# dropbox/divans

Measured on AMD Instinct MI355X. Metric: MB/s encode+decode per GPU, 64 KiB metablocks; bit-exact vs CPU, higher is better.
Workload: dtype u16/u64 integer

## Files before the change

divans_amd/csrc/capi.cpp:

```cpp
#include <hip/hip_runtime.h>

#include <algorithm>
#include <atomic>
#include <cstdio>
#include <cstdlib>
#include <cstring>
#include <mutex>
#include <string>
#include <vector>

#include "../../include/divans_gpu.h"
#include "lit_kernels.h"
#include "lit_device.h"

using namespace divans_hip;

static thread_local std::string g_last_error;
static int fail(int code, const std::string& msg) { g_last_error = msg; return code; }
#define HIP_TRY(expr)                                                                              \
    do {                                                                                           \
        hipError_t e_ = (expr);                                                                    \
        if (e_ != hipSuccess)                                                                      \
            return fail(DIVANS_GPU_EHIP, std::string(#expr) + ": " + hipGetErrorString(e_));       \
    } while (0)
// ... 916 lines not shown
            rc = after(s0, k.n_streams, view); if (rc) return rc;
        }
        return 0;
    }
    rc = ensure_sf(c, n_streams); if (rc) return rc;
    rc = ensure_tables(c); if (rc) return rc;
    LitBatch b;
    std::memset(&b, 0, sizeof(b));
    b.blob = c->d_blob; b.geom = c->geom; b.tables = c->d_tables;
    b.n_streams = n_streams; b.stream_len = stream_len; b.max_stream_len = c->max_stream_len;
    b.in = d_in; b.in_offsets = d_in_offsets; b.in_sizes = d_in_sizes;
    b.sf = c->d_sf; b.status = c->d_status;
    b.seg_begin = d_seg_begin; b.segs = (const LitSegment*)d_segs;
    set_cache_fields(c, b);
    if (d_segs && b.cache_mode != 2u && b.cache_mode != 0u) return fail(DIVANS_GPU_EINVAL, "segment lists need the default (high-nibble-row) cache or none");
    HIP_TRY(hipEventRecord(c->ev[0], c->stream));
    ++c->table_launch_seq;
    HIP_TRY(launch_model_encode(b, c->mix, c->blocks, c->stream));
    view.sf = c->d_sf; view.stride = 2u * c->max_stream_len;
    return after(0u, n_streams, view);
}

static int rans_event_pair(divans_gpu_codec* c, size_t i, hipEvent_t*& pair) {
    while (c->ev_rans.size() < 2u * (i + 1u)) {
        hipEvent_t e = nullptr;
        HIP_TRY(hipEventCreate(&e));
        c->ev_rans.push_back(e);
    }
    pair = &c->ev_rans[2u * i];
    return 0;
}

static int rans_pass(divans_gpu_codec* c, const SfView& v, uint32_t count, uint32_t stream_len, const uint32_t* d_in_sizes, uint8_t* out, uint64_t out_base,
                     uint64_t out_slot, uint64_t* d_out_offsets, uint32_t* d_out_sizes, uint32_t* d_chunk_bytes, uint32_t max_chunks, size_t& pairs) {
    const bool chunk_lanes = c->max_stream_len > 32768u && c->max_stream_len <= 65536u;
    RansBatch r;
    r.sf = v.sf; r.sf_stride = v.stride; r.n_streams = count; r.stream_len = stream_len; r.max_stream_len = c->max_stream_len;
    r.in_sizes = d_in_sizes;
    r.out = out; r.out_base = out_base; r.out_slot = out_slot;
    r.out_offsets = d_out_offsets; r.out_sizes = d_out_sizes;
    r.status = c->d_status; r.chunk_bytes = d_chunk_bytes; r.max_chunks = max_chunks;
    r.scratch = nullptr; r.scratch_stride = 0; r.chunk0_sizes = nullptr;
    if (chunk_lanes) { int rr = ensure_rans_scratch(c, count, v, r); if (rr) return rr; }
    r.split_states = (c->rans_split == 2u || (c->rans_split == 0u && (uint64_t)count * 4u <= (uint64_t)c->num_cus * 4u * 64u)) ? 1u : 0u;
    hipEvent_t* pair = nullptr;
    int rr = rans_event_pair(c, pairs, pair); if (rr) return rr;
    HIP_TRY(hipEventRecord(pair[0], c->stream));
    HIP_TRY(launch_rans_encode(r, c->stream));
    HIP_TRY(hipEventRecord(pair[1], c->stream));
    ++pairs;
    return 0;
}

static int encode_batch_impl(divans_gpu_codec* c, const uint8_t* d_in, const uint64_t* d_in_offsets,
                             const uint32_t* d_in_sizes, uint32_t stream_len, uint32_t n_streams,
                             uint8_t* d_out, uint64_t out_slot, uint64_t* d_out_offsets, uint32_t* d_out_sizes,
                             uint32_t* d_chunk_bytes, uint32_t max_chunks,
                             const uint32_t* d_seg_begin = nullptr, const divans_lit_segment* d_segs = nullptr);

extern "C" int divans_gpu_lit_encode_batch(divans_gpu_codec* c, const uint8_t* d_in, const uint64_t* d_in_offsets,
                                           const uint32_t* d_in_sizes, uint32_t stream_len, uint32_t n_streams,
                                           uint8_t* d_out, uint64_t out_slot, uint64_t* d_out_offsets, uint32_t* d_out_sizes) {
    return encode_batch_impl(c, d_in, d_in_offsets, d_in_sizes, stream_len, n_streams, d_out, out_slot, d_out_offsets,
                             d_out_sizes, nullptr, 0);
}

static int encode_batch_impl(divans_gpu_codec* c, const uint8_t* d_in, const uint64_t* d_in_offsets,
                             const uint32_t* d_in_sizes, uint32_t stream_len, uint32_t n_streams,
                             uint8_t* d_out, uint64_t out_slot, uint64_t* d_out_offsets, uint32_t* d_out_sizes,
                             uint32_t* d_chunk_bytes, uint32_t max_chunks,
                             const uint32_t* d_seg_begin, const divans_lit_segment* d_segs) {
    if (!c || !d_in || !d_out || !d_out_offsets || !d_out_sizes) return fail(DIVANS_GPU_EINVAL, "null argument");
    if ((d_seg_begin == nullptr) != (d_segs == nullptr)) return fail(DIVANS_GPU_EINVAL, "seg_begin and segs go together");
    if (n_streams == 0) return 0;
    if ((d_in_offsets == nullptr) != (d_in_sizes == nullptr)) return fail(DIVANS_GPU_EINVAL, "offsets and sizes go together");
    if (stream_len > c->max_stream_len) return fail(DIVANS_GPU_EINVAL, "stream_len exceeds the codec's max_stream_len");
// ... 11 lines not shown
    c->rans_pairs = pairs; c->enc_spans = 0;
    c->timing_pending_enc = true;
    return 0;
}

extern "C" int divans_gpu_lit_encode_packed(divans_gpu_codec* c, const uint8_t* d_in, const uint64_t* d_in_offsets, const uint32_t* d_in_sizes,
                                            uint32_t stream_len, uint32_t n_streams, uint8_t* d_packed, uint64_t packed_cap,
                                            uint64_t* d_packed_offsets, uint32_t* d_sizes, uint64_t* d_total, uint32_t sub_batch) {
    if (!c || !d_in || !d_packed || !d_packed_offsets || !d_sizes || !d_total) return fail(DIVANS_GPU_EINVAL, "null argument");
    if ((d_in_offsets == nullptr) != (d_in_sizes == nullptr)) return fail(DIVANS_GPU_EINVAL, "offsets and sizes go together");
    if (stream_len > c->max_stream_len) return fail(DIVANS_GPU_EINVAL, "stream_len exceeds the codec's max_stream_len");
    HIP_TRY(hipSetDevice(c->device));
    HIP_TRY(hipMemsetAsync(d_total, 0, sizeof(uint64_t), c->stream));
    if (n_streams == 0) return 0;
    const uint64_t slot = divans_gpu_lit_encode_bound(d_in_sizes ? c->max_stream_len : stream_len);
    uint32_t sub = std::min(n_streams, sub_batch ? sub_batch : c->bucket_mix_batch);
    while ((uint64_t)sub * slot > ((uint64_t)1 << 36) && sub > 1024u) sub = (sub + 1u) / 2u;
    if ((size_t)sub * slot > c->slots_bytes) {
        if (c->d_slots) { HIP_TRY(hipStreamSynchronize(c->stream)); HIP_TRY(hipFree(c->d_slots)); c->d_slots = nullptr; c->slots_bytes = 0; }
        if (device_alloc((void**)&c->d_slots, (size_t)sub * slot) != hipSuccess) return fail(DIVANS_GPU_ENOMEM, "hipMalloc(output slots of a sub-batch) failed");
        c->slots_bytes = (size_t)sub * slot;
    }
    if (sub > c->slot_off_cap) {
        if (c->d_slot_off) { HIP_TRY(hipStreamSynchronize(c->stream)); HIP_TRY(hipFree(c->d_slot_off)); c->d_slot_off = nullptr; c->slot_off_cap = 0; }
        if (hipMalloc(&c->d_slot_off, (size_t)sub * sizeof(uint64_t)) != hipSuccess) return fail(DIVANS_GPU_ENOMEM, "hipMalloc(slot offsets) failed");
        c->slot_off_cap = sub;
    }
    const size_t n_sub = (n_streams + sub - 1u) / sub;
    while (c->ev_span.size() < 3u * n_sub) { hipEvent_t e = nullptr; HIP_TRY(hipEventCreate(&e)); c->ev_span.push_back(e); }
    size_t pairs = 0, span = 0;
    for (uint32_t b0 = 0; b0 < n_streams; b0 += sub, ++span) {
        const uint32_t m = std::min(sub, n_streams - b0);
        HIP_TRY(hipEventRecord(c->ev_span[3u * span], c->stream));
        int rc = model_pass(c, d_in_offsets ? d_in : d_in + (size_t)b0 * stream_len, d_in_offsets ? d_in_offsets + b0 : nullptr, d_in_sizes ? d_in_sizes + b0 : nullptr,
                            stream_len, m, nullptr, nullptr, [&](uint32_t first, uint32_t count, const SfView& v) -> int {
            return rans_pass(c, v, count, stream_len, d_in_sizes ? d_in_sizes + b0 + first : nullptr, c->d_slots + (uint64_t)first * slot, (uint64_t)first * slot, slot,
                             c->d_slot_off + first, d_sizes + b0 + first, nullptr, 0, pairs);
        });
        if (rc) return rc;
        HIP_TRY(hipEventRecord(c->ev_span[3u * span + 1u], c->stream));
        HIP_TRY(launch_pack(c->d_slots, c->d_slot_off, d_sizes + b0, m, d_packed, d_packed_offsets + b0, d_total, c->stream, true, packed_cap, c->d_status));
        HIP_TRY(hipEventRecord(c->ev_span[3u * span + 2u], c->stream));
    }
    c->rans_pairs = pairs; c->enc_spans = span;
    c->timing_pending_enc = true;
    return 0;
}

extern "C" int divans_gpu_lit_encode_batch_chunks(divans_gpu_codec* c, const uint8_t* d_in, const uint64_t* d_in_offsets,
                                                  const uint32_t* d_in_sizes, uint32_t stream_len, uint32_t n_streams,
                                                  uint8_t* d_out, uint64_t out_slot, uint64_t* d_out_offsets, uint32_t* d_out_sizes,
                                                  uint32_t* d_chunk_bytes, uint32_t max_chunks) {
    if (!d_chunk_bytes || max_chunks < (2u * (uint64_t)stream_len + 65535u) / 65536u) return fail(DIVANS_GPU_EINVAL, "max_chunks too small");
    return encode_batch_impl(c, d_in, d_in_offsets, d_in_sizes, stream_len, n_streams, d_out, out_slot, d_out_offsets, d_out_sizes,
                             d_chunk_bytes, max_chunks);
}

extern "C" int divans_gpu_lit_encode_segments_batch(divans_gpu_codec* c, const uint8_t* d_in, const uint64_t* d_in_offsets,
                                                    const uint32_t* d_in_sizes, uint32_t stream_len, uint32_t n_streams,
                                                    const uint32_t* d_seg_begin, const divans_lit_segment* d_segs,
                                                    uint8_t* d_out, uint64_t out_slot, uint64_t* d_out_offsets, uint32_t* d_out_sizes) {
    if (!d_seg_begin || !d_segs) return fail(DIVANS_GPU_EINVAL, "null segment list");
    return encode_batch_impl(c, d_in, d_in_offsets, d_in_sizes, stream_len, n_streams, d_out, out_slot, d_out_offsets,
                             d_out_sizes, nullptr, 0, d_seg_begin, d_segs);
}

extern "C" int divans_gpu_lit_model_batch(divans_gpu_codec* c, const uint8_t* d_in, const uint64_t* d_in_offsets,
                                          const uint32_t* d_in_sizes, uint32_t stream_len, uint32_t n_streams, uint32_t* d_pairs) {
    if (!c || !d_in || !d_pairs) return fail(DIVANS_GPU_EINVAL, "null argument");
    if (n_streams == 0) return 0;
    if ((d_in_offsets == nullptr) != (d_in_sizes == nullptr)) return fail(DIVANS_GPU_EINVAL, "offsets and sizes go together");
    if (stream_len > c->max_stream_len) return fail(DIVANS_GPU_EINVAL, "stream_len exceeds the codec's max_stream_len");
    HIP_TRY(hipSetDevice(c->device));
    const size_t row = (size_t)2u * c->max_stream_len * sizeof(uint32_t);
// ... 782 lines not shown
```

divans_amd/csrc/lit_kernels.h:

```cpp
#ifndef DIVANS_LIT_KERNELS_H_
#define DIVANS_LIT_KERNELS_H_
#include <hip/hip_runtime.h>
#include <stdint.h>

namespace divans_hip {

constexpr int LIT_THREADS = 256;
constexpr int RANS_THREADS = 64;

constexpr uint32_t LIT_BLOB_LUT1CLASS = 0;
constexpr uint32_t LIT_BLOB_CTXF = 256;
constexpr uint32_t LIT_CTXF_BYTES = 2048;
constexpr uint32_t LIT_MAX_BTYPES = 8;
constexpr uint32_t LIT_BLOB_MAX_BYTES = 256 + LIT_CTXF_BYTES * LIT_MAX_BTYPES + 8192;

struct LitGeometry {
    uint32_t nctx;
    uint32_t low_width;
    uint32_t plane0, plane1, plane2;
    uint32_t low_base;
    uint32_t cm_base;
    uint32_t total_rows;
    int32_t mm_uniform;
    int32_t ctx_const;
// ... 10 lines not shown
struct LitBatch {
    const uint8_t* blob;
    LitGeometry geom;
    int16_t* tables;
    uint32_t n_streams, stream_len, max_stream_len;
    const uint8_t* in; const uint64_t* in_offsets; const uint32_t* in_sizes;
    uint8_t* out; const uint64_t* out_offsets; const uint32_t* out_sizes;
    uint32_t* sf;
    uint32_t cache_rows_high;
    uint32_t cache_rows_low;
    uint32_t cache_mode;
    uint32_t cache_bytes_per_wg;
    const uint32_t* seg_begin;
    const LitSegment* segs;
    uint32_t* status;
    uint32_t dm_log2, dm_shift;
    uint8_t* stream_bad;
    uint32_t resume; int32_t* wstate;
    uint32_t* consumed;
    const uint8_t* byte_rank;
};
constexpr uint32_t LIT_STATUS_BAD_MODEL = 1u;
constexpr uint32_t LIT_STATUS_BAD_SEGMENT = 4u;
constexpr uint32_t LIT_STATUS_OUTPUT_FULL = 8u;
constexpr uint32_t LIT_STATUS_BAD_STREAM = 2u;

struct RansBatch {
    const uint32_t* sf; uint32_t n_streams, stream_len, max_stream_len; const uint32_t* in_sizes;
    uint32_t sf_stride;
    uint64_t out_base;
    uint8_t* out; uint64_t out_slot; uint64_t* out_offsets; uint32_t* out_sizes; uint32_t* status;
    uint32_t* chunk_bytes; uint32_t max_chunks;
    uint8_t* scratch; uint64_t scratch_stride; uint32_t* chunk0_sizes;
    uint32_t split_states;
};

typedef unsigned int bk_u32x2 __attribute__((ext_vector_type(2)));
struct BucketBatch {
    const uint8_t* in; const uint64_t* in_offsets; const uint32_t* in_sizes;
    uint32_t n_streams, stream_len, max_stream_len;
    uint32_t pieces;
    uint32_t slot;
    uint32_t sf_stride;
    uint8_t* sorted;
    uint16_t* inv;
    uint32_t* desc;
    bk_u32x2* sfs;
    uint32_t* sf;
    uint32_t* tasks;
    uint32_t* counters;
    int32_t inc, lim;
};
hipError_t launch_bucket_model(const BucketBatch& b, uint32_t chain_blocks, hipStream_t st);
void launch_bucket_tasks(const BucketBatch& b, hipStream_t st);
void launch_bucket_unsort(const BucketBatch& b, hipStream_t st);
void launch_bucket_unsort32(const BucketBatch& b, hipStream_t st);

struct MixBucketBatch {
    const uint8_t* in; const uint64_t* in_offsets; const uint32_t* in_sizes;
    uint32_t n_streams, stream_len, max_stream_len;
    uint32_t pieces;
    uint32_t slot;
    uint32_t pos_stride;
    uint32_t sf_stride;
    const uint8_t* blob;
    uint16_t* sorted;
    uint16_t* inv;
    uint32_t* desc;
    uint32_t* tasks;
    uint32_t* counters;
    bk_u32x2* xs[2];
    uint32_t* maxes[2];
    uint32_t* sf;
    int32_t inc0, lim0, inc2, lim2, inc3, lim3;
};
hipError_t launch_bucket_mix_model(const MixBucketBatch& b, uint32_t num_cus, hipStream_t st);

uint32_t lit_lds_bytes(const LitBatch& b);
hipError_t launch_model_encode(const LitBatch& b, bool mix, uint32_t blocks, hipStream_t st);
hipError_t launch_rans_encode(const RansBatch& b, hipStream_t st);
hipError_t launch_decode(const LitBatch& b, bool mix, uint32_t blocks, hipStream_t st);
hipError_t launch_decode2(const LitBatch& b, bool mix, uint32_t blocks, hipStream_t st);
void lit_decode_kernel_name(const LitBatch& b, bool mix, char* buf, size_t cap);
void lit_decode2_kernel_name(const LitBatch& b, bool mix, char* buf, size_t cap);
uint32_t lit_decode2_effective_caches(uint32_t dm_log2, bool mix, bool seg);
uint32_t lit_decode2_stream_lds(uint32_t dm_log2);
#ifndef DIVANS_WITH_EXPERIMENTAL_DECODERS
#define DIVANS_WITH_EXPERIMENTAL_DECODERS 0
#endif
#if DIVANS_WITH_EXPERIMENTAL_DECODERS
hipError_t launch_decode_t(const LitBatch& b, bool mix, uint32_t blocks, hipStream_t st);
hipError_t launch_selftest_cdf_ops_t(const uint32_t* d_ops, uint32_t n, int32_t* d_out, hipStream_t st);
void lit_decode_t_kernel_name(const LitBatch& b, bool mix, char* buf, size_t cap);
uint32_t lit_decode_t_stream_lds(uint32_t dm_log2, bool mix);
#endif
hipError_t launch_pack(const uint8_t* slots, const uint64_t* src_off, const uint32_t* sizes, uint32_t n, uint8_t* packed,
                       uint64_t* dst_off, uint64_t* total, hipStream_t st, bool accumulate = false, uint64_t cap = ~0ull, uint32_t* status = nullptr);
hipError_t launch_learn_byte_rank(const uint8_t* data, const uint64_t* offsets, const uint32_t* sizes, uint32_t n_streams, uint32_t stream_len,
                                  uint32_t sample_streams, uint32_t sample_len, uint8_t* rank, hipStream_t st);
hipError_t launch_row_replay(const LitBatch& b, bool mix, uint32_t blocks, hipStream_t st);
hipError_t launch_selftest_division(unsigned long long* d_mismatches, hipStream_t st);
hipError_t launch_selftest_cdf_ops(const uint32_t* d_ops, uint32_t n, int32_t* d_out, hipStream_t st);
hipError_t launch_selftest_cdf_ops2(const uint32_t* d_ops, uint32_t n, int32_t* d_out, hipStream_t st);
hipError_t launch_selftest_cdf_ops_bucket(const uint32_t* d_ops, uint32_t n, int32_t* d_out, hipStream_t st);

}
#endif
```

divans_amd/csrc/lit_kernels.hip:

```cpp
#include <hip/hip_runtime.h>
#include <stdio.h>
#include <stdint.h>

#include "lit_device.h"

namespace divans_hip {

struct RowRef { uint32_t row; uint32_t slot_addr; };
constexpr uint32_t kNoSlot = 0xffffffffu;

struct CacheDesc {
    uint32_t data_off;
    uint32_t tag_off;
    uint32_t set_mask;
};

template <int CACHE>
struct Table {
    __amdgpu_buffer_rsrc_t rsrc;
    uint32_t lane_off;
    uint8_t* lds;
    CacheDesc ch, cl;
    __device__ __forceinline__ int gload(uint32_t row) const {
        return (int)__builtin_amdgcn_raw_buffer_load_b16(rsrc, lane_off + (row << 5), 0, 0);
// ... 250 lines not shown
                    rowL = fetch_row<false, MM, CACHE>(g, lv, tb, ctx_cur, last8, nb >> 4);
                    cur = nb;
                    pend_a = (uint32_t)li == k ? ph : pend_a;
                    pend_b = (uint32_t)li == k ? pl : pend_b;
                }
            }
            if ((uint32_t)li < cnt) {
                u32x2 v = {pend_a, pend_b};
                __builtin_nontemporal_store(v, (u32x2*)(sf + 2u * (size_t)(base + li)));
            }
            mine = nxt;
            nxt = (base + 32u + li < len) ? in[base + 32u + li] : 0u;
        }
        if (SEG && li == 0) sc.finish();
        if (MIX && b.wstate && (li & 7) == 0) {
            int32_t* p = b.wstate + (li ? 3 : 0);
            p[0] = wp.w.w0; p[1] = wp.w.w1; p[2] = wp.w.norm;
        }
        if (g.wrap_check) {
            __builtin_amdgcn_fence(__ATOMIC_RELEASE, "workgroup");
            __builtin_amdgcn_s_waitcnt(0);
            if (wrap_scan<CACHE>(g, tb, li, rbase) && li == 0) {
                if (b.status) atomicOr(b.status, LIT_STATUS_BAD_MODEL);
                if (b.stream_bad) b.stream_bad[s] = 1;
            }
        }
    }
}

__device__ __forceinline__ void rans_store_word(uint32_t* p, uint32_t v) {
    asm volatile("global_store_dword %0, %1, off" : : "v"(p), "v"(v) : "memory");
}

#ifndef DIVANS_RANS_DIVMOD
#define DIVANS_RANS_DIVMOD 1
#endif
__device__ __forceinline__ uint64_t rans_divmod(uint64_t state, uint32_t freq, uint32_t& rem) {
    const double fd = (double)freq;
    double y = __builtin_amdgcn_rcp(fd);
    y = __builtin_fma(__builtin_fma(-fd, y, 1.0), y, y);
    y = __builtin_fma(__builtin_fma(-fd, y, 1.0), y, y);
#if DIVANS_RANS_DIVMOD
    y *= (1.0 - 0x1p-49);
    const double sd = __builtin_fma((double)(uint32_t)(state >> 32), 0x1p32, (double)(uint32_t)state);
    const double t = __builtin_trunc(sd * y) + 0x1p52;
    uint64_t q = (uint64_t)__builtin_bit_cast(unsigned long long, t) & ((1ull << 52) - 1ull);
#else
    y *= (1.0 - 0x1p-49);
    const double qd = (double)state * y;
    uint64_t q = (uint64_t)qd;
#endif
    uint32_t r = (uint32_t)state - (uint32_t)q * freq;
    if (r >= freq) { q += 1; r -= freq; }
    rem = r;
    return q;
}

__device__ __forceinline__ uint64_t rans_put(uint64_t state, uint32_t start, uint32_t freq, uint32_t*& wp) {
    if ((uint32_t)(state >> 32) >= (freq << 16)) { rans_store_word(--wp, (uint32_t)state); state >>= 32; }
    uint32_t r;
    const uint64_t q = rans_divmod(state, freq, r);
    return (q << 15) + (uint64_t)r + (uint64_t)start;
}

__device__ __forceinline__ uint32_t* rans_encode_chunk(const uint32_t* sf, uint32_t beg, uint32_t end, uint32_t* wp, uint32_t& bad) {
    uint64_t a = 1ull << 31, bst = 1ull << 31;
    uint32_t i = end;
    auto put = [&](uint32_t p) {
        const uint32_t start = p & 0xffffu;
        uint32_t freq = p >> 16;
        bad |= (freq == 0u) | (freq >> 15) | (start >> 15);
        freq = freq ? freq : 1u;
        const uint64_t x = rans_put(a, start, freq, wp);
        a = bst; bst = x;
    };
    while (i > beg && (i & 3u)) put(sf[--i]);
    struct Quad { u32x4 a, b, c, d; };
    auto sat = [](uint32_t x, uint32_t k) { return x >= k ? x - k : 0u; };
    auto request1 = [&](u32x4& q, uint32_t top) {
        const uint32_t* p = sf + (top >= beg + 4u ? top - 4u : beg);
        asm volatile("global_load_dwordx4 %0, %1, off" : "=v"(q) : "v"(p) : "memory");
    };
    auto request = [&](Quad& q, uint32_t top) {
        request1(q.a, top); request1(q.b, sat(top, 4u)); request1(q.c, sat(top, 8u)); request1(q.d, sat(top, 12u));
    };
    auto code = [&](const u32x4& g) { if (i > beg) { put(g.w); put(g.z); put(g.y); put(g.x); i -= 4u; } };
    Quad q0, q1, q2, q3;
    request(q0, i); request(q1, sat(i, 16u)); request(q2, sat(i, 32u)); request(q3, sat(i, 48u));
#define RANS_STEP(Q)    \
    {                                                                                   \
        asm volatile("s_waitcnt vmcnt(12)" : "+v"(Q.a), "+v"(Q.b), "+v"(Q.c), "+v"(Q.d) : : "memory"); \
        const uint32_t top = i;                                                         \
        code(Q.a); code(Q.b); code(Q.c); code(Q.d);                                     \
        request(Q, sat(top, 64u));                                                      \
    }
    while (i > beg) { RANS_STEP(q0) RANS_STEP(q1) RANS_STEP(q2) RANS_STEP(q3) }
#undef RANS_STEP
    asm volatile("s_waitcnt vmcnt(0)" : "+v"(q0.a), "+v"(q0.b), "+v"(q0.c), "+v"(q0.d), "+v"(q1.a), "+v"(q1.b), "+v"(q1.c), "+v"(q1.d) : : "memory");
    asm volatile("" : "+v"(q2.a), "+v"(q2.b), "+v"(q2.c), "+v"(q2.d), "+v"(q3.a), "+v"(q3.b), "+v"(q3.c), "+v"(q3.d) : : "memory");
    const uint64_t fa = bst, fb = a;
    rans_store_word(--wp, (uint32_t)(fb >> 32)); rans_store_word(--wp, (uint32_t)fb);
    rans_store_word(--wp, (uint32_t)(fa >> 32)); rans_store_word(--wp, (uint32_t)fa);
    return wp;
}

__global__ __launch_bounds__(RANS_THREADS) void rans_encode_kernel(const RansBatch b) {
    const uint32_t s = blockIdx.x * RANS_THREADS + threadIdx.x;
    if (s >= b.n_streams) return;
    const uint32_t len = b.in_sizes ? b.in_sizes[s] : b.stream_len;
    const uint32_t nsym = 2u * len;
    const uint32_t* sf = b.sf + (size_t)s * b.sf_stride;
    uint8_t* slot_end = b.out + (uint64_t)(s + 1) * b.out_slot;
    uint32_t* wp = (uint32_t*)slot_end;
    uint32_t* chunk_top = wp;
    uint32_t bad = 0;
    uint32_t nchunks = (nsym + 65535u) >> 16;
    for (uint32_t ck = nchunks; ck-- > 0;) {
        const uint32_t beg = ck << 16;
        const uint32_t end = beg + 65536u < nsym ? beg + 65536u : nsym;
        wp = rans_encode_chunk(sf, beg, end, wp, bad);
        if (b.chunk_bytes) {
            b.chunk_bytes[(size_t)s * b.max_chunks + ck] = (uint32_t)((uint8_t*)chunk_top - (uint8_t*)wp);
            chunk_top = wp;
        }
    }
    uint64_t off = (uint64_t)((uint8_t*)wp - b.out) + b.out_base;
    b.out_offsets[s] = off;
    b.out_sizes[s] = (uint32_t)(slot_end - (uint8_t*)wp);
    if (bad) atomicOr(b.status, LIT_STATUS_BAD_MODEL);
}

__device__ __forceinline__ int pair_swap(int v) { return __builtin_amdgcn_mov_dpp(v, 0xb1 , 0xf, 0xf, false); }

__device__ __forceinline__ uint32_t rans_encode_chunk_split(const uint32_t* sf, uint32_t beg, uint32_t end, uint32_t* top, uint32_t second, uint32_t& bad) {
    uint64_t st = 1ull << 31;
    uint32_t cnt = 0;
    uint32_t i = end;
    auto put2 = [&](uint32_t pa, uint32_t pb) {
        const uint32_t p = second ? pb : pa;
        const uint32_t start = p & 0xffffu;
        uint32_t freq = p >> 16;
        bad |= (freq == 0u) | (freq >> 15) | (start >> 15);
        freq = freq ? freq : 1u;
        const uint32_t mine = (uint32_t)(st >> 32) >= (freq << 16) ? 1u : 0u;
        const uint32_t theirs = (uint32_t)pair_swap((int)mine);
        if (mine) { rans_store_word(top - 1u - cnt - (second ? theirs : 0u), (uint32_t)st); st >>= 32; }
        cnt += mine + theirs;
        uint32_t r;
        const uint64_t q = rans_divmod(st, freq, r);
        st = (q << 15) + (uint64_t)r + (uint64_t)start;
    };
    if (i > beg && (i & 3u)) { put2(sf[i - 1u], sf[i - 2u]); i -= 2u; }
    struct Quad { u32x4 a, b, c, d; };
    auto sat = [](uint32_t x, uint32_t k) { return x >= k ? x - k : 0u; };
    auto request1 = [&](u32x4& q, uint32_t t) {
        const uint32_t* p = sf + (t >= beg + 4u ? t - 4u : beg);
        asm volatile("global_load_dwordx4 %0, %1, off" : "=v"(q) : "v"(p) : "memory");
    };
    auto request = [&](Quad& q, uint32_t t) { request1(q.a, t); request1(q.b, sat(t, 4u)); request1(q.c, sat(t, 8u)); request1(q.d, sat(t, 12u)); };
    auto code = [&](const u32x4& g) { if (i > beg) { put2(g.w, g.z); put2(g.y, g.x); i -= 4u; } };
    Quad q0, q1, q2, q3;
    request(q0, i); request(q1, sat(i, 16u)); request(q2, sat(i, 32u)); request(q3, sat(i, 48u));
#define RANS_STEP(Q)                                                                    \
    {                                                                                   \
        asm volatile("s_waitcnt vmcnt(12)" : "+v"(Q.a), "+v"(Q.b), "+v"(Q.c), "+v"(Q.d) : : "memory"); \
        const uint32_t t0 = i;                                                          \
        code(Q.a); code(Q.b); code(Q.c); code(Q.d);                                     \
        request(Q, sat(t0, 64u));                                                       \
    }
    while (i > beg) { RANS_STEP(q0) RANS_STEP(q1) RANS_STEP(q2) RANS_STEP(q3) }
#undef RANS_STEP
    asm volatile("s_waitcnt vmcnt(0)" : "+v"(q0.a), "+v"(q0.b), "+v"(q0.c), "+v"(q0.d), "+v"(q1.a), "+v"(q1.b), "+v"(q1.c), "+v"(q1.d) : : "memory");
    asm volatile("" : "+v"(q2.a), "+v"(q2.b), "+v"(q2.c), "+v"(q2.d), "+v"(q3.a), "+v"(q3.b), "+v"(q3.c), "+v"(q3.d) : : "memory");
    uint32_t* wp = top - cnt - (second ? 4u : 2u);
    rans_store_word(wp, (uint32_t)st); rans_store_word(wp + 1, (uint32_t)(st >> 32));
    return 4u * (cnt + 4u);
}

__global__ __launch_bounds__(256) __attribute__((amdgpu_waves_per_eu(2, 2))) void rans_encode2_split_kernel(const RansBatch b) {
    const uint32_t g = blockIdx.x * 256u + threadIdx.x;
    const uint32_t s = g >> 2, ck = (g >> 1) & 1u, second = g & 1u;
    const bool live = s < b.n_streams;
    const uint32_t len = live ? (b.in_sizes ? b.in_sizes[s] : b.stream_len) : 0u;
    const uint32_t nsym = 2u * len, beg = ck << 16;
    uint8_t* slot_end = b.out + (uint64_t)(s + 1) * b.out_slot;
    uint32_t size = 0, bad = 0;
    if (live && beg < nsym) {
        const uint32_t end = beg + 65536u < nsym ? beg + 65536u : nsym;
        const uint32_t* sf = b.sf + (size_t)s * b.sf_stride;
        uint8_t* top = ck ? slot_end : b.scratch + (uint64_t)(s + 1) * b.scratch_stride;
        size = rans_encode_chunk_split(sf, beg, end, (uint32_t*)top, second, bad);
        if (b.chunk_bytes && !second) b.chunk_bytes[(size_t)s * b.max_chunks + ck] = size;
    }
    const uint32_t other = (uint32_t)__shfl_xor((int)size, 2);
    if (live && (g & 3u) == 0u) {
        const uint32_t total = size + other;
        b.out_sizes[s] = total;
        b.out_offsets[s] = (uint64_t)(slot_end - b.out) - total + b.out_base;
        b.chunk0_sizes[s] = size;
    }
    if (bad) atomicOr(b.status, LIT_STATUS_BAD_MODEL);
}

#ifndef DIVANS_RANS2_THREADS
#define DIVANS_RANS2_THREADS 256
#endif
constexpr int RANS2_THREADS = DIVANS_RANS2_THREADS;
__global__ __launch_bounds__(RANS2_THREADS) __attribute__((amdgpu_waves_per_eu(2, 2))) void rans_encode2_kernel(const RansBatch b) {
// ... 204 lines not shown
            __builtin_amdgcn_fence(__ATOMIC_RELEASE, "workgroup");
            __builtin_amdgcn_s_waitcnt(0);
            corrupt |= wrap_scan<CACHE>(g, tb, li, rbase);
        }
        if (corrupt && li == 0) {
            if (b.status) atomicOr(b.status, LIT_STATUS_BAD_STREAM);
            if (b.stream_bad) b.stream_bad[s] = 1;
        }
    }
}

__global__ __launch_bounds__(1024) void scan_sizes_kernel(const uint32_t* sizes, uint32_t n, uint64_t* offsets, uint64_t* total, int accumulate) {
    __shared__ uint64_t partial[1024];
    const uint32_t t = threadIdx.x;
    const uint64_t base = accumulate ? *total : 0ull;
    const uint32_t per = (n + 1023u) / 1024u;
    const uint32_t beg = t * per < n ? t * per : n, end = beg + per < n ? beg + per : n;
    uint64_t sum = 0;
    for (uint32_t i = beg; i < end; ++i) sum += (sizes[i] + 3u) & ~3u;
    partial[t] = sum;
    __syncthreads();
    for (uint32_t off = 1; off < 1024u; off <<= 1) {
        uint64_t v = t >= off ? partial[t - off] : 0;
        __syncthreads();
        partial[t] += v;
        __syncthreads();
    }
    uint64_t run = base + (t ? partial[t - 1] : 0);
    for (uint32_t i = beg; i < end; ++i) { offsets[i] = run; run += (sizes[i] + 3u) & ~3u; }
    if (t == 1023u) *total = base + partial[1023];
}

__global__ __launch_bounds__(256) void pack_copy_kernel(const uint8_t* slots, const uint64_t* src_off, const uint32_t* sizes,
                                                        uint32_t n, uint8_t* packed, const uint64_t* dst_off, uint64_t cap, uint32_t* status) {
    const uint32_t wave = (blockIdx.x * 256u + threadIdx.x) >> 6, lane = threadIdx.x & 63u;
    const uint32_t nw = (gridDim.x * 256u) >> 6;
    for (uint32_t s = wave; s < n; s += nw) {
        const uint32_t* src = (const uint32_t*)(slots + src_off[s]);
        uint32_t* dst = (uint32_t*)(packed + dst_off[s]);
        const uint32_t words = (sizes[s] + 3u) >> 2;
        if (dst_off[s] + 4ull * words > cap) {
            if (lane == 0 && status) atomicOr(status, LIT_STATUS_OUTPUT_FULL);
            continue;
        }
        for (uint32_t i = lane; i < words; i += 64u) dst[i] = src[i];
    }
}

__global__ void selftest_division_kernel(unsigned long long* mismatches) {
    unsigned long long bad = 0;
    for (uint32_t mx = blockIdx.x + 1; mx < 32768u; mx += gridDim.x) {
        float rcp = __builtin_amdgcn_rcpf((float)mx);
        for (uint32_t c = threadIdx.x; c <= mx; c += blockDim.x) {
            uint32_t n = c << 15;
            bad += exact_div(n, mx, rcp) != n / mx;
            bad += scaled_div((int)c, (int)mx, biased_rcp15((int)mx)) != n / mx;
        }
        for (uint32_t k = threadIdx.x; k < 4096u; k += blockDim.x) {
            const uint64_t top = (uint64_t)mx << 48;
            uint64_t x = (uint64_t)k * 0x9E3779B97F4A7C15ull + (uint64_t)mx * 0xD1B54A32D192ED03ull;
            x ^= x >> 29;
            const uint64_t cand[6] = {top - 1ull - k, (x % top), (x % top) / mx * mx, ((x % top) / mx * mx) + mx - 1ull,
                                      (1ull << 31) + k * 977ull, (x >> (k & 31)) % top};
            for (int j = 0; j < 6; ++j) {
                uint32_t rem;
                const uint64_t q = rans_divmod(cand[j], mx, rem);
                bad += (q != cand[j] / mx) | (rem != (uint32_t)(cand[j] % mx));
            }
        }
    }
    if (bad) atomicAdd(mismatches, bad);
}

__global__ __launch_bounds__(64) void cdf_ops_selftest_kernel(const u32x4* ops, uint32_t n, int32_t* out) {
    const int lane = threadIdx.x & 63, li = lane & 15, rbase = lane & 48;
    int c0 = 4 * (li + 1), c1 = 4 * (li + 1);
    Weights w = {1, 1, 1 << 14};
    for (uint32_t k = 0; k < n; ++k) {
        const u32x4 op = ops[k];
        int rec = 0;
        switch (op.x) {
        case 0: c0 = blend_row(c0, li, (int)op.y, (int)op.z, (int)op.w); rec = c0; break;
        case 1: c1 = blend_row(c1, li, (int)op.y, (int)op.z, (int)op.w); rec = c1; break;
        case 2: rec = average_rows(c0, c1, row_bcast<15>(c0), row_bcast<15>(c1), (int)op.y); break;
        case 3: case 4: {
            const int mx = row_bcast<15>(c0);
            const int sym = op.x == 3 ? (int)op.y : search_symbol(c0, op.y & 0x7fffu, rbase);
            const uint32_t d = scaled_div(c0, mx, biased_rcp15(mx));
            const int dprev = row_prev_or_zero((int)d);
            const uint32_t sf = (uint32_t)(dprev + 1) | ((uint32_t)((int)d - dprev - 1) << 16);
            const uint32_t packed = (uint32_t)row_gather((int)sf, rbase, sym);
            rec = li == 0 ? (int)(packed & 0xffffu) : (li == 1 ? (int)(packed >> 16) : (li == 2 ? sym : 0));
            break;
        }
        case 5: weights_update(w, (int)(short)op.y, (int)(short)op.z, (int)(short)op.w);
                rec = li == 0 ? w.w0 : (li == 1 ? w.w1 : (li == 2 ? w.norm : 0)); break;
        case 6: c0 = 4 * (li + 1); c1 = 4 * (li + 1); w.w0 = 1; w.w1 = 1; w.norm = 1 << 14; rec = c0; break;
        case 7: c0 = blend_row_known_max(c0, li, (int)op.y, (int)op.z, (int)op.w, row_bcast<15>(c0)); rec = c0; break;
        case 8:
            if (op.y == 0u) { c0 = li == (int)(op.z & 15u) ? (int)(short)op.w : c0; rec = c0; }
            else if (op.y == 1u) { c1 = li == (int)(op.z & 15u) ? (int)(short)op.w : c1; rec = c1; }
// ... 81 lines not shown
    if (seg) return cache_mode == 2 ? pick_lit_decode_kernel<2, true>(mm, ctxc, mix) : pick_lit_decode_kernel<0, true>(mm, ctxc, mix);
    if (cache_mode == 2) return pick_lit_decode_kernel<2, false>(mm, ctxc, mix);
    return cache_mode == 0 ? pick_lit_decode_kernel<0, false>(mm, ctxc, mix) : nullptr;
}
#endif

static int effective_mm(int mm) { return (mm == 0 || mm == 4) ? mm : -1; }

uint32_t lit_lds_bytes(const LitBatch& b) {
    uint32_t bytes = b.cache_bytes_per_wg;
    if (b.geom.ctx_const < 0) bytes += LIT_BLOB_CTXF + LIT_CTXF_BYTES * b.geom.n_btypes;
    if (effective_mm(b.geom.mm_uniform) < 0) bytes += 8192u;
    return bytes;
}

hipError_t launch_model_encode(const LitBatch& b_in, bool mix, uint32_t blocks, hipStream_t st) {
    const LitBatch& b = b_in;
    const int mm = effective_mm(b.geom.mm_uniform);
    if (b.segs && b.cache_mode != 2u && b.cache_mode != 0u) return hipErrorInvalidValue;
    LitKernel k = pick_mode_lit_model_encode_kernel((int)b.cache_mode, b.segs != nullptr, mm, b.geom.ctx_const >= 0, mix);
    const uint32_t lds = lit_lds_bytes(b);
    if (lds > 65536u) (void)hipFuncSetAttribute((const void*)k, hipFuncAttributeMaxDynamicSharedMemorySize, (int)lds);
    hipLaunchKernelGGL(k, dim3(blocks), dim3(LIT_THREADS), lds, st, b);
    return hipGetLastError();
}
hipError_t launch_rans_encode(const RansBatch& b, hipStream_t st) {
    if (b.scratch) {
        if (b.split_states) {
            hipLaunchKernelGGL(rans_encode2_split_kernel, dim3((4u * b.n_streams + 255u) / 256u), dim3(256), 0, st, b);
        } else {
            const uint32_t blocks = (2u * b.n_streams + RANS2_THREADS - 1) / RANS2_THREADS;
            hipLaunchKernelGGL(rans_encode2_kernel, dim3(blocks), dim3(RANS2_THREADS), 0, st, b);
        }
        const uint32_t sblocks = (b.n_streams + 3u) / 4u < 8192u ? (b.n_streams + 3u) / 4u : 8192u;
        hipLaunchKernelGGL(rans_stitch_kernel, dim3(sblocks), dim3(256), 0, st, b);
        return hipGetLastError();
    }
    uint32_t blocks = (b.n_streams + RANS_THREADS - 1) / RANS_THREADS;
    hipLaunchKernelGGL(rans_encode_kernel, dim3(blocks), dim3(RANS_THREADS), 0, st, b);
    return hipGetLastError();
}
void lit_decode_kernel_name(const LitBatch& b, bool mix, char* buf, size_t cap) {
    const int mm = effective_mm(b.geom.mm_uniform);
    const bool seg = b.segs != nullptr;
    const int cache = seg ? (b.cache_mode == 2u ? 2 : 0) : (b.cache_mode >= 1u && b.cache_mode <= 3u ? (int)b.cache_mode : 0);
    snprintf(buf, cap, "divans_hip::lit_decode_kernel<%d, %s, %s, %d, %s>", mm, b.geom.ctx_const >= 0 ? "true" : "false", mix ? "true" : "false", cache,
             seg ? "true" : "false");
}
hipError_t launch_decode(const LitBatch& b_in, bool mix, uint32_t blocks, hipStream_t st) {
    const LitBatch& b = b_in;
    const int mm = effective_mm(b.geom.mm_uniform);
    if (b.segs && b.cache_mode != 2u && b.cache_mode != 0u) return hipErrorInvalidValue;
    LitKernel k = pick_mode_lit_decode_kernel((int)b.cache_mode, b.segs != nullptr, mm, b.geom.ctx_const >= 0, mix);
    if (!k) return hipErrorInvalidValue;
    const uint32_t lds = lit_lds_bytes(b);
    if (lds > 65536u) (void)hipFuncSetAttribute((const void*)k, hipFuncAttributeMaxDynamicSharedMemorySize, (int)lds);
    hipLaunchKernelGGL(k, dim3(blocks), dim3(LIT_THREADS), lds, st, b);
    return hipGetLastError();
}
hipError_t launch_pack(const uint8_t* slots, const uint64_t* src_off, const uint32_t* sizes, uint32_t n, uint8_t* packed,
                       uint64_t* dst_off, uint64_t* total, hipStream_t st, bool accumulate, uint64_t cap, uint32_t* status) {
    hipLaunchKernelGGL(scan_sizes_kernel, dim3(1), dim3(1024), 0, st, sizes, n, dst_off, total, accumulate ? 1 : 0);
    uint32_t blocks = (n + 3) / 4;
    blocks = blocks > 2048 ? 2048 : (blocks ? blocks : 1);
    hipLaunchKernelGGL(pack_copy_kernel, dim3(blocks), dim3(256), 0, st, slots, src_off, sizes, n, packed, dst_off, cap, status);
    return hipGetLastError();
}
hipError_t launch_selftest_cdf_ops(const uint32_t* d_ops, uint32_t n, int32_t* d_out, hipStream_t st) {
    hipLaunchKernelGGL(cdf_ops_selftest_kernel, dim3(1), dim3(64), 0, st, (const u32x4*)d_ops, n, d_out);
    return hipGetLastError();
}
hipError_t launch_selftest_division(unsigned long long* d_mismatches, hipStream_t st) {
    hipLaunchKernelGGL(selftest_division_kernel, dim3(1024), dim3(256), 0, st, d_mismatches);
    return hipGetLastError();
}

}
```

Measured before the change: 15290.

## Split rANS state into 32-bit halves, batch validity checks, fuse stitch into pack

The rANS encoder now holds its state as two 32-bit halves and uses a branchless advance step that folds the remainder correction into a min/select. Validity checks on symbol words are accumulated once per quad instead of once per symbol. When the whole sub-batch goes through one rANS pass with chunk lanes, the separate stitch kernel is skipped and the pack copy reads chunk 0 directly from scratch, which removes one kernel launch and one copy pass. The division self-test is extended to cover the new advance step at edge cases.

```diff
diff --git a/divans_amd/csrc/capi.cpp b/divans_amd/csrc/capi.cpp
--- a/divans_amd/csrc/capi.cpp
+++ b/divans_amd/csrc/capi.cpp
@@ -972,7 +972,8 @@
 }
 
 static int rans_pass(divans_gpu_codec* c, const SfView& v, uint32_t count, uint32_t stream_len, const uint32_t* d_in_sizes, uint8_t* out, uint64_t out_base,
-                     uint64_t out_slot, uint64_t* d_out_offsets, uint32_t* d_out_sizes, uint32_t* d_chunk_bytes, uint32_t max_chunks, size_t& pairs) {
+                     uint64_t out_slot, uint64_t* d_out_offsets, uint32_t* d_out_sizes, uint32_t* d_chunk_bytes, uint32_t max_chunks, size_t& pairs,
+                     PackChunk0* unstitched = nullptr) {
     const bool chunk_lanes = c->max_stream_len > 32768u && c->max_stream_len <= 65536u;
     RansBatch r;
     r.sf = v.sf; r.sf_stride = v.stride; r.n_streams = count; r.stream_len = stream_len; r.max_stream_len = c->max_stream_len;
@@ -980,8 +981,12 @@
     r.out = out; r.out_base = out_base; r.out_slot = out_slot;
     r.out_offsets = d_out_offsets; r.out_sizes = d_out_sizes;
     r.status = c->d_status; r.chunk_bytes = d_chunk_bytes; r.max_chunks = max_chunks;
-    r.scratch = nullptr; r.scratch_stride = 0; r.chunk0_sizes = nullptr;
+    r.scratch = nullptr; r.scratch_stride = 0; r.chunk0_sizes = nullptr; r.defer_stitch = 0;
     if (chunk_lanes) { int rr = ensure_rans_scratch(c, count, v, r); if (rr) return rr; }
+    if (unstitched) {
+        if (chunk_lanes) { r.defer_stitch = 1; *unstitched = PackChunk0{r.scratch, r.scratch_stride, r.chunk0_sizes}; }
+        else *unstitched = PackChunk0{nullptr, 0, nullptr};
+    }
     r.split_states = (c->rans_split == 2u || (c->rans_split == 0u && (uint64_t)count * 4u <= (uint64_t)c->num_cus * 4u * 64u)) ? 1u : 0u;
     hipEvent_t* pair = nullptr;
     int rr = rans_event_pair(c, pairs, pair); if (rr) return rr;
@@ -1059,14 +1064,16 @@
     for (uint32_t b0 = 0; b0 < n_streams; b0 += sub, ++span) {
         const uint32_t m = std::min(sub, n_streams - b0);
         HIP_TRY(hipEventRecord(c->ev_span[3u * span], c->stream));
+        PackChunk0 chunk0{nullptr, 0, nullptr};
         int rc = model_pass(c, d_in_offsets ? d_in : d_in + (size_t)b0 * stream_len, d_in_offsets ? d_in_offsets + b0 : nullptr, d_in_sizes ? d_in_sizes + b0 : nullptr,
                             stream_len, m, nullptr, nullptr, [&](uint32_t first, uint32_t count, const SfView& v) -> int {
             return rans_pass(c, v, count, stream_len, d_in_sizes ? d_in_sizes + b0 + first : nullptr, c->d_slots + (uint64_t)first * slot, (uint64_t)first * slot, slot,
-                             c->d_slot_off + first, d_sizes + b0 + first, nullptr, 0, pairs);
+                             c->d_slot_off + first, d_sizes + b0 + first, nullptr, 0, pairs, first == 0u && count == m ? &chunk0 : nullptr);
         });
         if (rc) return rc;
         HIP_TRY(hipEventRecord(c->ev_span[3u * span + 1u], c->stream));
-        HIP_TRY(launch_pack(c->d_slots, c->d_slot_off, d_sizes + b0, m, d_packed, d_packed_offsets + b0, d_total, c->stream, true, packed_cap, c->d_status));
+        HIP_TRY(launch_pack(c->d_slots, c->d_slot_off, d_sizes + b0, m, d_packed, d_packed_offsets + b0, d_total, c->stream, true, packed_cap, c->d_status,
+                            chunk0.sizes ? &chunk0 : nullptr));
         HIP_TRY(hipEventRecord(c->ev_span[3u * span + 2u], c->stream));
     }
     c->rans_pairs = pairs; c->enc_spans = span;
diff --git a/divans_amd/csrc/lit_kernels.h b/divans_amd/csrc/lit_kernels.h
--- a/divans_amd/csrc/lit_kernels.h
+++ b/divans_amd/csrc/lit_kernels.h
@@ -66,6 +66,7 @@
     uint8_t* out; uint64_t out_slot; uint64_t* out_offsets; uint32_t* out_sizes; uint32_t* status;
     uint32_t* chunk_bytes; uint32_t max_chunks;
     uint8_t* scratch; uint64_t scratch_stride; uint32_t* chunk0_sizes;
+    uint32_t defer_stitch;
     uint32_t split_states;
 };
 
@@ -128,8 +129,10 @@
 void lit_decode_t_kernel_name(const LitBatch& b, bool mix, char* buf, size_t cap);
 uint32_t lit_decode_t_stream_lds(uint32_t dm_log2, bool mix);
 #endif
+struct PackChunk0 { const uint8_t* scratch; uint64_t stride; const uint32_t* sizes; };
 hipError_t launch_pack(const uint8_t* slots, const uint64_t* src_off, const uint32_t* sizes, uint32_t n, uint8_t* packed,
-                       uint64_t* dst_off, uint64_t* total, hipStream_t st, bool accumulate = false, uint64_t cap = ~0ull, uint32_t* status = nullptr);
+                       uint64_t* dst_off, uint64_t* total, hipStream_t st, bool accumulate = false, uint64_t cap = ~0ull, uint32_t* status = nullptr,
+                       const PackChunk0* chunk0 = nullptr);
 hipError_t launch_learn_byte_rank(const uint8_t* data, const uint64_t* offsets, const uint32_t* sizes, uint32_t n_streams, uint32_t stream_len,
                                   uint32_t sample_streams, uint32_t sample_len, uint8_t* rank, hipStream_t st);
 hipError_t launch_row_replay(const LitBatch& b, bool mix, uint32_t blocks, hipStream_t st);
diff --git a/divans_amd/csrc/lit_kernels.hip b/divans_amd/csrc/lit_kernels.hip
--- a/divans_amd/csrc/lit_kernels.hip
+++ b/divans_amd/csrc/lit_kernels.hip
@@ -306,49 +306,97 @@
     asm volatile("global_store_dword %0, %1, off" : : "v"(p), "v"(v) : "memory");
 }
 
-#ifndef DIVANS_RANS_DIVMOD
-#define DIVANS_RANS_DIVMOD 1
+#ifndef DIVANS_RANS_QUOTIENT_FMA
+#define DIVANS_RANS_QUOTIENT_FMA 0
 #endif
-__device__ __forceinline__ uint64_t rans_divmod(uint64_t state, uint32_t freq, uint32_t& rem) {
+#ifndef DIVANS_RANS_QUAD_VALIDITY
+#define DIVANS_RANS_QUAD_VALIDITY 1
+#endif
+__device__ __forceinline__ uint64_t rans_quotient_bits(uint32_t lo, uint32_t hi, uint32_t freq) {
     const double fd = (double)freq;
     double y = __builtin_amdgcn_rcp(fd);
     y = __builtin_fma(__builtin_fma(-fd, y, 1.0), y, y);
-    y = __builtin_fma(__builtin_fma(-fd, y, 1.0), y, y);
-#if DIVANS_RANS_DIVMOD
-    y *= (1.0 - 0x1p-49);
-    const double sd = __builtin_fma((double)(uint32_t)(state >> 32), 0x1p32, (double)(uint32_t)state);
+    y = __builtin_fma(__builtin_fma(-fd, y, 1.0 - 0x1p-49), y, y);
+    const double sd = __builtin_fma((double)hi, 0x1p32, (double)lo);
+#if DIVANS_RANS_QUOTIENT_FMA
+    const double t = __builtin_fma(sd, y, 0x1p52 - 0.5);
+#else
     const double t = __builtin_trunc(sd * y) + 0x1p52;
-    uint64_t q = (uint64_t)__builtin_bit_cast(unsigned long long, t) & ((1ull << 52) - 1ull);
+#endif
+    return (uint64_t)__builtin_bit_cast(unsigned long long, t);
+}
+
+#ifndef DIVANS_RANS_PUSH_ASM
+#define DIVANS_RANS_PUSH_ASM 0
+#endif
+__device__ __forceinline__ void rans_store_word_if(uint32_t* p, uint32_t v, bool push) {
+#if DIVANS_RANS_PUSH_ASM
+    unsigned long long saved;
+    const unsigned long long m = __builtin_amdgcn_ballot_w64(push);
+    asm volatile("s_and_saveexec_b64 %0, %1\n\tglobal_store_dword %2, %3, off\n\ts_mov_b64 exec, %0"
+                 : "=&s"(saved) : "s"(m), "v"(p), "v"(v) : "memory", "scc");
 #else
-    y *= (1.0 - 0x1p-49);
-    const double qd = (double)state * y;
-    uint64_t q = (uint64_t)qd;
+    if (push) rans_store_word(p, v);
 #endif
+}
+__device__ __forceinline__ void rans_push_word_if(uint32_t*& wp, uint32_t v, bool push) {
+#if DIVANS_RANS_PUSH_ASM
+    unsigned long long saved;
+    const unsigned long long m = __builtin_amdgcn_ballot_w64(push);
+    asm volatile("s_and_saveexec_b64 %0, %2\n\tv_lshl_add_u64 %1, %1, 0, -4\n\tglobal_store_dword %1, %3, off\n\ts_mov_b64 exec, %0"
+                 : "=&s"(saved), "+v"(wp) : "s"(m), "v"(v) : "memory", "scc");
+#else
+    if (push) rans_store_word(--wp, v);
+#endif
+}
+
+__device__ __forceinline__ uint64_t rans_divmod(uint64_t state, uint32_t freq, uint32_t& rem) {
+    uint64_t q = rans_quotient_bits((uint32_t)state, (uint32_t)(state >> 32), freq) & ((1ull << 52) - 1ull);
     uint32_t r = (uint32_t)state - (uint32_t)q * freq;
     if (r >= freq) { q += 1; r -= freq; }
     rem = r;
     return q;
 }
 
-__device__ __forceinline__ uint64_t rans_put(uint64_t state, uint32_t start, uint32_t freq, uint32_t*& wp) {
-    if ((uint32_t)(state >> 32) >= (freq << 16)) { rans_store_word(--wp, (uint32_t)state); state >>= 32; }
-    uint32_t r;
-    const uint64_t q = rans_divmod(state, freq, r);
-    return (q << 15) + (uint64_t)r + (uint64_t)start;
+__device__ __forceinline__ void rans_advance(uint32_t& lo, uint32_t& hi, uint32_t start, uint32_t freq) {
+    const uint64_t qb = rans_quotient_bits(lo, hi, freq);
+    const uint32_t r = lo - (uint32_t)qb * freq;
+    const uint32_t t = r - freq;
+    const uint32_t u = (r < t ? r : t) + start + (r >= freq ? 0x8000u : 0u);
+    const uint64_t x = (qb << 15) + (uint64_t)u;
+    lo = (uint32_t)x; hi = (uint32_t)(x >> 32);
+}
+
+__device__ __forceinline__ void rans_shift_out(uint32_t& lo, uint32_t& hi, bool push) {
+    lo = push ? hi : lo;
+    hi = push ? 0u : hi;
+}
+
+struct RansSym { uint32_t start, freq, lim; };
+__device__ __forceinline__ RansSym rans_sym(uint32_t p) {
+    p = p < 0x10000u ? 0x10000u : p;
+    return {p & 0xffffu, p >> 16, p & 0xffff0000u};
+}
+__device__ __forceinline__ uint32_t rans_pair_bad(uint32_t p) { return (p < 0x10000u) | ((p & 0x80008000u) != 0u); }
+
+__device__ __forceinline__ void rans_put(uint32_t& lo, uint32_t& hi, uint32_t p, uint32_t*& wp) {
+    const RansSym y = rans_sym(p);
+    const bool push = hi >= y.lim;
+    rans_push_word_if(wp, lo, push);
+    rans_shift_out(lo, hi, push);
+    rans_advance(lo, hi, y.start, y.freq);
 }
 
 __device__ __forceinline__ uint32_t* rans_encode_chunk(const uint32_t* sf, uint32_t beg, uint32_t end, uint32_t* wp, uint32_t& bad) {
-    uint64_t a = 1ull << 31, bst = 1ull << 31;
+    uint32_t alo = 1u << 31, ahi = 0u, blo = 1u << 31, bhi = 0u;
     uint32_t i = end;
     auto put = [&](uint32_t p) {
-        const uint32_t start = p & 0xffffu;
-        uint32_t freq = p >> 16;
-        bad |= (freq == 0u) | (freq >> 15) | (start >> 15);
-        freq = freq ? freq : 1u;
-        const uint64_t x = rans_put(a, start, freq, wp);
-        a = bst; bst = x;
+        rans_put(alo, ahi, p, wp);
+        const uint32_t tl = alo, th = ahi;
+        alo = blo; ahi = bhi; blo = tl; bhi = th;
     };
-    while (i > beg && (i & 3u)) put(sf[--i]);
+    while (i > beg && (i & 3u)) { const uint32_t p = sf[--i]; bad |= rans_pair_bad(p); put(p); }
+    uint32_t any = 0u, least = ~0u;
     struct Quad { u32x4 a, b, c, d; };
     auto sat = [](uint32_t x, uint32_t k) { return x >= k ? x - k : 0u; };
     auto request1 = [&](u32x4& q, uint32_t top) {
@@ -358,7 +406,17 @@
     auto request = [&](Quad& q, uint32_t top) {
         request1(q.a, top); request1(q.b, sat(top, 4u)); request1(q.c, sat(top, 8u)); request1(q.d, sat(top, 12u));
     };
-    auto code = [&](const u32x4& g) { if (i > beg) { put(g.w); put(g.z); put(g.y); put(g.x); i -= 4u; } };
+    auto code = [&](const u32x4& g) {
+        if (i > beg) {
+#if DIVANS_RANS_QUAD_VALIDITY
+            any |= g.x | g.y | g.z | g.w;
+            least = min(least, min(min(g.x, g.y), min(g.z, g.w)));
+#else
+            bad |= rans_pair_bad(g.x) | rans_pair_bad(g.y) | rans_pair_bad(g.z) | rans_pair_bad(g.w);
+#endif
+            put(g.w); put(g.z); put(g.y); put(g.x); i -= 4u;
+        }
+    };
     Quad q0, q1, q2, q3;
     request(q0, i); request(q1, sat(i, 16u)); request(q2, sat(i, 32u)); request(q3, sat(i, 48u));
 #define RANS_STEP(Q)    \
@@ -372,9 +430,9 @@
 #undef RANS_STEP
     asm volatile("s_waitcnt vmcnt(0)" : "+v"(q0.a), "+v"(q0.b), "+v"(q0.c), "+v"(q0.d), "+v"(q1.a), "+v"(q1.b), "+v"(q1.c), "+v"(q1.d) : : "memory");
     asm volatile("" : "+v"(q2.a), "+v"(q2.b), "+v"(q2.c), "+v"(q2.d), "+v"(q3.a), "+v"(q3.b), "+v"(q3.c), "+v"(q3.d) : : "memory");
-    const uint64_t fa = bst, fb = a;
-    rans_store_word(--wp, (uint32_t)(fb >> 32)); rans_store_word(--wp, (uint32_t)fb);
-    rans_store_word(--wp, (uint32_t)(fa >> 32)); rans_store_word(--wp, (uint32_t)fa);
+    bad |= ((any & 0x80008000u) != 0u) | (least < 0x10000u);
+    rans_store_word(--wp, ahi); rans_store_word(--wp, alo);
+    rans_store_word(--wp, bhi); rans_store_word(--wp, blo);
     return wp;
 }
 
@@ -407,24 +465,25 @@
 __device__ __forceinline__ int pair_swap(int v) { return __builtin_amdgcn_mov_dpp(v, 0xb1 , 0xf, 0xf, false); }
 
 __device__ __forceinline__ uint32_t rans_encode_chunk_split(const uint32_t* sf, uint32_t beg, uint32_t end, uint32_t* top, uint32_t second, uint32_t& bad) {
-    uint64_t st = 1ull << 31;
+    uint32_t lo = 1u << 31, hi = 0u;
     uint32_t cnt = 0;
     uint32_t i = end;
     auto put2 = [&](uint32_t pa, uint32_t pb) {
         const uint32_t p = second ? pb : pa;
-        const uint32_t start = p & 0xffffu;
-        uint32_t freq = p >> 16;
-        bad |= (freq == 0u) | (freq >> 15) | (start >> 15);
-        freq = freq ? freq : 1u;
-        const uint32_t mine = (uint32_t)(st >> 32) >= (freq << 16) ? 1u : 0u;
+        const RansSym y = rans_sym(p);
+        const uint32_t mine = hi >= y.lim ? 1u : 0u;
         const uint32_t theirs = (uint32_t)pair_swap((int)mine);
-        if (mine) { rans_store_word(top - 1u - cnt - (second ? theirs : 0u), (uint32_t)st); st >>= 32; }
+        rans_store_word_if(top - 1u - cnt - (second ? theirs : 0u), lo, mine != 0u);
+        rans_shift_out(lo, hi, mine != 0u);
         cnt += mine + theirs;
-        uint32_t r;
-        const uint64_t q = rans_divmod(st, freq, r);
-        st = (q << 15) + (uint64_t)r + (uint64_t)start;
+        rans_advance(lo, hi, y.start, y.freq);
     };
-    if (i > beg && (i & 3u)) { put2(sf[i - 1u], sf[i - 2u]); i -= 2u; }
+    uint32_t any = 0u, least = ~0u;
+    if (i > beg && (i & 3u)) {
+        const uint32_t pa = sf[i - 1u], pb = sf[i - 2u];
+        bad |= rans_pair_bad(pa) | rans_pair_bad(pb);
+        put2(pa, pb); i -= 2u;
+    }
     struct Quad { u32x4 a, b, c, d; };
     auto sat = [](uint32_t x, uint32_t k) { return x >= k ? x - k : 0u; };
     auto request1 = [&](u32x4& q, uint32_t t) {
@@ -432,7 +491,17 @@
         asm volatile("global_load_dwordx4 %0, %1, off" : "=v"(q) : "v"(p) : "memory");
     };
     auto request = [&](Quad& q, uint32_t t) { request1(q.a, t); request1(q.b, sat(t, 4u)); request1(q.c, sat(t, 8u)); request1(q.d, sat(t, 12u)); };
-    auto code = [&](const u32x4& g) { if (i > beg) { put2(g.w, g.z); put2(g.y, g.x); i -= 4u; } };
+    auto code = [&](const u32x4& g) {
+        if (i > beg) {
+#if DIVANS_RANS_QUAD_VALIDITY
+            any |= g.x | g.y | g.z | g.w;
+            least = min(least, min(min(g.x, g.y), min(g.z, g.w)));
+#else
+            bad |= rans_pair_bad(g.x) | rans_pair_bad(g.y) | rans_pair_bad(g.z) | rans_pair_bad(g.w);
+#endif
+            put2(g.w, g.z); put2(g.y, g.x); i -= 4u;
+        }
+    };
     Quad q0, q1, q2, q3;
     request(q0, i); request(q1, sat(i, 16u)); request(q2, sat(i, 32u)); request(q3, sat(i, 48u));
 #define RANS_STEP(Q)                                                                    \
@@ -446,8 +515,9 @@
 #undef RANS_STEP
     asm volatile("s_waitcnt vmcnt(0)" : "+v"(q0.a), "+v"(q0.b), "+v"(q0.c), "+v"(q0.d), "+v"(q1.a), "+v"(q1.b), "+v"(q1.c), "+v"(q1.d) : : "memory");
     asm volatile("" : "+v"(q2.a), "+v"(q2.b), "+v"(q2.c), "+v"(q2.d), "+v"(q3.a), "+v"(q3.b), "+v"(q3.c), "+v"(q3.d) : : "memory");
+    bad |= ((any & 0x80008000u) != 0u) | (least < 0x10000u);
     uint32_t* wp = top - cnt - (second ? 4u : 2u);
-    rans_store_word(wp, (uint32_t)st); rans_store_word(wp + 1, (uint32_t)(st >> 32));
+    rans_store_word(wp, lo); rans_store_word(wp + 1, hi);
     return 4u * (cnt + 4u);
 }
 
@@ -718,7 +788,8 @@
 }
 
 __global__ __launch_bounds__(256) void pack_copy_kernel(const uint8_t* slots, const uint64_t* src_off, const uint32_t* sizes,
-                                                        uint32_t n, uint8_t* packed, const uint64_t* dst_off, uint64_t cap, uint32_t* status) {
+                                                        uint32_t n, uint8_t* packed, const uint64_t* dst_off, uint64_t cap, uint32_t* status,
+                                                        const PackChunk0 chunk0) {
     const uint32_t wave = (blockIdx.x * 256u + threadIdx.x) >> 6, lane = threadIdx.x & 63u;
     const uint32_t nw = (gridDim.x * 256u) >> 6;
     for (uint32_t s = wave; s < n; s += nw) {
@@ -729,8 +800,20 @@
             if (lane == 0 && status) atomicOr(status, LIT_STATUS_OUTPUT_FULL);
             continue;
         }
-        for (uint32_t i = lane; i < words; i += 64u) dst[i] = src[i];
-    }
+        const uint32_t words0 = chunk0.sizes ? chunk0.sizes[s] >> 2 : 0u;
+        const uint32_t* src0 = (const uint32_t*)(chunk0.scratch + (uint64_t)(s + 1) * chunk0.stride) - words0;
+        for (uint32_t i = lane; i < words; i += 64u) dst[i] = i < words0 ? src0[i] : src[i];
+    }
+}
+
+__device__ __forceinline__ unsigned long long rans_step_differs(uint64_t state, uint32_t mx, uint32_t salt) {
+    uint32_t rem;
+    const uint64_t q = rans_divmod(state, mx, rem);
+    const uint32_t start = salt % (32769u - mx);
+    uint32_t lo = (uint32_t)state, hi = (uint32_t)(state >> 32);
+    rans_advance(lo, hi, start, mx);
+    const uint64_t want = ((state / mx) << 15) + state % mx + start;
+    return (unsigned long long)((q != state / mx) | (rem != (uint32_t)(state % mx)) | (lo != (uint32_t)want) | (hi != (uint32_t)(want >> 32)));
 }
 
 __global__ void selftest_division_kernel(unsigned long long* mismatches) {
@@ -748,11 +831,18 @@
             x ^= x >> 29;
             const uint64_t cand[6] = {top - 1ull - k, (x % top), (x % top) / mx * mx, ((x % top) / mx * mx) + mx - 1ull,
                                       (1ull << 31) + k * 977ull, (x >> (k & 31)) % top};
-            for (int j = 0; j < 6; ++j) {
-                uint32_t rem;
-                const uint64_t q = rans_divmod(cand[j], mx, rem);
-                bad += (q != cand[j] / mx) | (rem != (uint32_t)(cand[j] % mx));
+            for (int j = 0; j < 6; ++j) bad += rans_step_differs(cand[j], mx, k);
+        }
+        if (threadIdx.x < 64u) {
+            const uint64_t k = threadIdx.x, top = (uint64_t)mx << 48, qmax = (top - 1ull) / mx;
+            const uint64_t qs[3] = {0xffffffffull, 1ull << 32, qmax};
+            uint64_t cand[16] = {(1ull << 31) + (k << 25), (1ull << 32) - 1ull - k, 1ull << 32, (1ull << 32) + 1ull + k,
+                                 top - (1ull << 32) * (k + 1ull), top - (1ull << 32) * k - 1ull, top - 1ull};
+            for (int j = 0; j < 3; ++j) {
+                const uint64_t m = (qs[j] - (j == 2 ? k : 0ull)) * mx;
+                cand[7 + 3 * j] = m - 1ull; cand[8 + 3 * j] = m; cand[9 + 3 * j] = m + mx - 1ull;
             }
+            for (int j = 0; j < 16; ++j) bad += rans_step_differs(cand[j], mx, (uint32_t)k * 521u);
         }
     }
     if (bad) atomicAdd(mismatches, bad);
@@ -900,6 +990,7 @@
             const uint32_t blocks = (2u * b.n_streams + RANS2_THREADS - 1) / RANS2_THREADS;
             hipLaunchKernelGGL(rans_encode2_kernel, dim3(blocks), dim3(RANS2_THREADS), 0, st, b);
         }
+        if (b.defer_stitch) return hipGetLastError();
         const uint32_t sblocks = (b.n_streams + 3u) / 4u < 8192u ? (b.n_streams + 3u) / 4u : 8192u;
         hipLaunchKernelGGL(rans_stitch_kernel, dim3(sblocks), dim3(256), 0, st, b);
         return hipGetLastError();
@@ -927,11 +1018,12 @@
     return hipGetLastError();
 }
 hipError_t launch_pack(const uint8_t* slots, const uint64_t* src_off, const uint32_t* sizes, uint32_t n, uint8_t* packed,
-                       uint64_t* dst_off, uint64_t* total, hipStream_t st, bool accumulate, uint64_t cap, uint32_t* status) {
+                       uint64_t* dst_off, uint64_t* total, hipStream_t st, bool accumulate, uint64_t cap, uint32_t* status, const PackChunk0* chunk0) {
     hipLaunchKernelGGL(scan_sizes_kernel, dim3(1), dim3(1024), 0, st, sizes, n, dst_off, total, accumulate ? 1 : 0);
     uint32_t blocks = (n + 3) / 4;
     blocks = blocks > 2048 ? 2048 : (blocks ? blocks : 1);
-    hipLaunchKernelGGL(pack_copy_kernel, dim3(blocks), dim3(256), 0, st, slots, src_off, sizes, n, packed, dst_off, cap, status);
+    hipLaunchKernelGGL(pack_copy_kernel, dim3(blocks), dim3(256), 0, st, slots, src_off, sizes, n, packed, dst_off, cap, status,
+                       chunk0 ? *chunk0 : PackChunk0{nullptr, 0, nullptr});
     return hipGetLastError();
 }
 hipError_t launch_selftest_cdf_ops(const uint32_t* d_ops, uint32_t n, int32_t* d_out, hipStream_t st) {
```

Result: no change. 15360 (median of 6 runs) (+0.5%).
